# Hfx-J/SGTD

Measured on AMD Instinct MI355X. Metric: query frames/sec vs map size (descriptor build + candidate selection), higher is better.
Workload: dtype f64

## Files before the change

sgtd_amd/csrc/common.hip.h:

```cpp
#pragma once
#include <hip/hip_runtime.h>
#include <stdint.h>

#define SGTD_WAVE 64
#define SGTD_MAX_K 16
#define SGTD_NCELL 27
#define SGTD_MAX_CAND 64

typedef unsigned long long u64;
typedef unsigned int u32;

struct DevCfg {
  int K;
  int tpi;
  int cand_num;
  double min_len, max_len, scale, rough;
};

__device__ __forceinline__ int lane_id() { return threadIdx.x & (SGTD_WAVE - 1); }

__device__ __forceinline__ u64 lanemask_lt() {
  return (1ull << lane_id()) - 1ull;
}

// ... 138 lines not shown
typedef float f32x2 __attribute__((ext_vector_type(2)));

struct HashSlot {
  u64 key;
  u32 bucket;
  u32 len;
};
#define SGTD_EMPTY_KEY 0xFFFFFFFFFFFFFFFFull

__device__ __forceinline__ u32 wave_incl_scan(u32 v) {
  int x = (int)v;
  x += __builtin_amdgcn_update_dpp(0, x, 0x111, 0xf, 0xf, false);
  x += __builtin_amdgcn_update_dpp(0, x, 0x112, 0xf, 0xf, false);
  x += __builtin_amdgcn_update_dpp(0, x, 0x114, 0xf, 0xf, false);
  x += __builtin_amdgcn_update_dpp(0, x, 0x118, 0xf, 0xf, false);
  x += __builtin_amdgcn_update_dpp(0, x, 0x142, 0xa, 0xf, false);
  x += __builtin_amdgcn_update_dpp(0, x, 0x143, 0xc, 0xf, false);
  return (u32)x;
}

__device__ __forceinline__ u32 wave_sum(u32 v) {
  return (u32)__builtin_amdgcn_readlane((int)wave_incl_scan(v), SGTD_WAVE - 1);
}

__device__ __forceinline__ u32 wave_max_u32(u32 v) {
  int x = (int)v;
#define SGTD_MAX_STEP(ctrl, rows) { const u32 o = (u32)__builtin_amdgcn_update_dpp(0, x, ctrl, rows, 0xf, false); x = (int)((u32)x > o ? (u32)x : o); }
  SGTD_MAX_STEP(0x111, 0xf) SGTD_MAX_STEP(0x112, 0xf) SGTD_MAX_STEP(0x114, 0xf) SGTD_MAX_STEP(0x118, 0xf)
  SGTD_MAX_STEP(0x142, 0xa) SGTD_MAX_STEP(0x143, 0xc)
#undef SGTD_MAX_STEP
  return (u32)__builtin_amdgcn_readlane(x, SGTD_WAVE - 1);
}

template <int BITS>
__device__ __forceinline__ void wave_group_rank(u32 digit, bool valid, u32 &rank, u32 &count) {
  u64 m = __ballot(valid);
#pragma unroll
  for (int b = 0; b < BITS; b++) {
    u64 bal = __ballot((digit >> b) & 1u);
    m &= ((digit >> b) & 1u) ? bal : ~bal;
  }
  rank = __popcll(m & lanemask_lt());
  count = __popcll(m);
}
```

sgtd_amd/csrc/probe_kernels.hip.h:

```cpp
#pragma once
#include "common.hip.h"
#include <type_traits>

struct TableView {
  const HotEntry *ent;
  IdMap map;
  const double *cold_side;
  const BucketDir *dir;
  const HashSlot *hash;
  u32 hash_mask;
  u32 n_entries;
  u32 frame_lo;
  u32 frame_span;
  u32 coarse_at;
  u32 whole_at;
  u32 tail_off;
  const BucketDir *dir1;
  const HashSlot *hash1;
  u32 hash_mask1;
  u32 n_entries1;
};
__host__ __device__ __forceinline__ u32 group_row_bytes(const TableView &T) { return T.tail_off ? 2u * SGTD_GROUP_ROW_BYTES : SGTD_GROUP_ROW_BYTES; }

struct QueryView {
// ... 80 lines not shown
  for (int q0 = 0; q0 < n_queries; q0 += 256) {
    const int q = q0 + threadIdx.x;
    const u32 v = (q < n_queries) ? count[q] : 0;
    u32 tot;
    const u32 ex = block_excl_scan(v, lds, tot);
    if (q < n_queries) q_prefix[q] = carry + ex;
    carry += tot;
  }
  if (threadIdx.x == 0) *n_valid = carry;
}

__device__ __forceinline__ u64 home_coord(double s, u64 cmask) {
  return (int)(s - 1.0) < 0 ? cmask : min((u64)(u32)(int)s, cmask);
}

template <class KeyT>
__global__ void home_keys_kernel(QueryView Q, const u32 *q_prefix, KeyT *keys, u32 *vals, long long n_slots,
                                 int cbits, int sub_bits) {
  const long long d = (long long)blockIdx.x * blockDim.x + threadIdx.x;
  if (d >= n_slots) return;
  const int q = (int)(d / Q.stride);
  const u32 i = (u32)(d - (long long)q * Q.stride);
  if (i >= Q.count[q]) return;
  const u64 code = label_code(Q.label[d * 3 + 0], Q.label[d * 3 + 1], Q.label[d * 3 + 2]);
  const u64 cmask = (1ull << cbits) - 1ull;
  const u64 x = home_coord(Q.side[d * 3 + 0], cmask), y = home_coord(Q.side[d * 3 + 1], cmask),
            z = home_coord(Q.side[d * 3 + 2], cmask);
  const u32 idx = q_prefix[q] + i;
  const int ny = 1 << (sub_bits >> 1), nz = 1 << (sub_bits - (sub_bits >> 1));
  const double f1 = Q.side[d * 3 + 1] - (double)(int)Q.side[d * 3 + 1], f2 = Q.side[d * 3 + 2] - (double)(int)Q.side[d * 3 + 2];
  const u64 sub = (u64)min(max((int)(f1 * ny), 0), ny - 1) * nz + (u64)min(max((int)(f2 * nz), 0), nz - 1);
  keys[idx] = (KeyT)(((((code << cbits | x) << cbits | y) << cbits) | z) << sub_bits | sub);
  vals[idx] = (u32)d;
}

template <class KeyT>
__global__ void group_heads_kernel(const KeyT *keys, const u32 *n_valid_p, u32 *flags, long long n, int cbits, int sub_bits) {
  const long long p = (long long)blockIdx.x * blockDim.x + threadIdx.x;
  if (p >= n) return;
  u32 head = 0;
  if (p + 1 < (long long)*n_valid_p) {
    const u64 a = (u64)keys[p + 1] >> sub_bits, b = (u64)keys[p] >> sub_bits;
    const u64 cmask = (1ull << cbits) - 1ull;
    head = (a != b) || ((a & cmask) == cmask) || (((a >> cbits) & cmask) == cmask) ||
           (((a >> (2 * cbits)) & cmask) == cmask);
  }
  flags[p] = head;
}

__global__ void group_first_kernel(const u32 *gid, const u32 *n_valid_p, u32 *group_first, u32 *n_groups, long long n) {
  const long long p = (long long)blockIdx.x * blockDim.x + threadIdx.x;
  const long long nv = (long long)*n_valid_p;
  if (p >= n || p >= nv) return;
  const u32 g = gid[p];
  if (p == 0 || gid[p - 1] != g) group_first[g] = (u32)p;
  if (p == nv - 1) *n_groups = g + 1;
}

__global__ __launch_bounds__(256) void group_resolve_kernel(TableView T, QueryView Q, const u32 *order,
                                                            const u32 *group_first, const u32 *n_groups_p,
                                                            const u32 *n_valid_p, unsigned char *rows, u32 rows_cap,
                                                            int *overflow) {
  const int c = (int)(threadIdx.x & 31);
  const long long stride = ((long long)gridDim.x * blockDim.x) >> 5;
  const long long n_groups = (*n_valid_p) ? (long long)*n_groups_p : 0;
  if (n_groups > (long long)rows_cap) {
    if (blockIdx.x == 0 && threadIdx.x == 0) overflow[0] = 1;
    return;
  }
  for (long long g = ((long long)blockIdx.x * blockDim.x + threadIdx.x) >> 5; g < n_groups; g += stride) {
    if (c >= SGTD_NCELL) continue;
    const long long d = (long long)order[group_first[g]];
    const double q0 = Q.side[d * 3 + 0], q1 = Q.side[d * 3 + 1], q2 = Q.side[d * 3 + 2];
    const u32 code = label_code(Q.label[d * 3 + 0], Q.label[d * 3 + 1], Q.label[d * 3 + 2]);
    const int ix = c / 9 - 1, iy = (c / 3) % 3 - 1, iz = c % 3 - 1;
    const bool nonneg = q0 >= 0.0 && q1 >= 0.0 && q2 >= 0.0;
    const int x = nonneg ? max((int)q0 + ix, 0) : (int)(q0 + (double)ix);
    const int y = nonneg ? max((int)q1 + iy, 0) : (int)(q1 + (double)iy);
    const int z = nonneg ? max((int)q2 + iz, 0) : (int)(q2 + (double)iz);
    const bool minus_one = nonneg && ((ix < 0 && (int)(q0 + (double)ix) < 0) || (iy < 0 && (int)(q1 + (double)iy) < 0) ||
                                      (iz < 0 && (int)(q2 + (double)iz) < 0));
    const bool probe = !minus_one && x >= 0 && y >= 0 && z >= 0 && x < 65536 && y < 65536 && z < 65536;
    const u64 key = probe ? pack_key(code, (u32)x, (u32)y, (u32)z) : 0ull;
    for (int sg = 0; sg < (T.tail_off ? 2 : 1); sg++) {
      const HashSlot *hash = sg ? T.hash1 : T.hash;
      const BucketDir *dir = sg ? T.dir1 : T.dir;
      const u32 mask = sg ? T.hash_mask1 : T.hash_mask;
      uint4 lo = make_uint4(0, 0, 0, 0), hi = make_uint4(0, 0, 0, 0);
      if (probe) {
// ... 15 lines not shown
      uint4 *out = reinterpret_cast<uint4 *>(rows + (size_t)g * group_row_bytes(T) + (size_t)sg * SGTD_GROUP_ROW_BYTES);
      if (hi.w != 0u) {
        const u32 r = 1u + 2u * (u32)__builtin_popcount(exh & ((1u << c) - 1u));
        out[r] = lo;
        out[r + 1] = hi;
      }
      if (c == 0) out[0] = make_uint4(exh, (u32)(ov >> sh) & 0x7FFFFFFu, 0u, 0u);
    }
  }
}

#define SGTD_NO_PASS 0xFFFFFFFFu
#define SGTD_PASS_HDR_WORDS (SGTD_PASS_KMAX == 4 ? 32 : 16)
#define SGTD_PASS_HDR_UNITS (SGTD_PASS_HDR_WORDS / 4)
#define SGTD_META_SENTINEL (((1u << SGTD_PASS_KMAX) - 1u) << 8)
enum { PH_SLOT = 0, PH_FRAME, PH_Q0, PH_Q1, PH_Q2, PH_LO2, PH_HI2 };
__host__ __device__ constexpr int pass_hdr_word(int field, int k) { return 2 + field * SGTD_PASS_KMAX + k; }
#define SGTD_PASS_SLACK_UNITS 64

struct __attribute__((packed, aligned(4))) RangeWords { u32 offc, dlc, meta; };

struct PassPool {
  uint4 *pool;
  u32 *rec_off;
  u32 *cursor;
  u32 cap;
};

__host__ __device__ __forceinline__ u32 pass_slot_count(u32 n_valid, u32 n_groups, bool pair) {
  if (!n_valid) return 0u;
  return pair ? n_groups + (n_valid + SGTD_PAIR - 1u) / SGTD_PAIR + 1u : n_valid;
}

__global__ void pass_slots_kernel(const u32 *gid, const u32 *group_first, const u32 *n_valid_p, u32 *pos_of_slot,
                                  long long n, int pair) {
  const long long p = (long long)blockIdx.x * blockDim.x + threadIdx.x;
  if (p >= n || p >= (long long)*n_valid_p) return;
  if (!pair) { pos_of_slot[p] = (u32)p; return; }
  const u32 g = gid[p], f = group_first[g];
  if ((((u32)p - f) % SGTD_PAIR) == 0u) pos_of_slot[g + (f + SGTD_PAIR - 1u) / SGTD_PAIR + ((u32)p - f) / SGTD_PAIR] = (u32)p;
}

#define SGTD_SMALL_SLOTS 8192
#define SGTD_SMALL_THREADS 1024
struct SmallOrder {
  u32 *ctr; u32 ctr_words;
  u32 *q_M; unsigned long long *q_P;
  u32 *votes; u32 *slot_of_words; u32 span;
  int *cand_frame, *cand_votes; int cand_num;
  u32 *q_prefix, *n_valid, *order, *gid, *group_first, *n_groups, *pos_of_slot;
  u32 n_slots, max_pass_slots;
  int cbits, sub_bits, pair, key_bits;
  QueryRec *qrec; u32 n_qrec; double rough;
};
__global__ __launch_bounds__(SGTD_SMALL_THREADS) void small_order_kernel(QueryView Q, SmallOrder S) {
  extern __shared__ __attribute__((aligned(16))) unsigned char s_raw[];
  u64 *s_key = reinterpret_cast<u64 *>(s_raw);
  u32 *s_gid = reinterpret_cast<u32 *>(s_raw + SGTD_SMALL_SLOTS * 8);
  u32 *s_first = s_gid + SGTD_SMALL_SLOTS;
  __shared__ u32 s_sum[SGTD_SMALL_THREADS / SGTD_WAVE + 1];
  __shared__ u32 s_cnt[4096];
  const u32 tid = threadIdx.x;
  for (u32 i = tid; i < S.ctr_words; i += SGTD_SMALL_THREADS) S.ctr[i] = 0u;
  if (tid == 0) { S.q_M[0] = 0u; S.q_P[0] = 0ull; S.q_prefix[0] = 0u; }
  if (S.votes) for (u32 i = tid; i < S.span; i += SGTD_SMALL_THREADS) S.votes[i] = 0u;
  if (S.slot_of_words) for (u32 i = tid; i < (S.span + 3u) / 4u; i += SGTD_SMALL_THREADS) S.slot_of_words[i] = 0xFFFFFFFFu;
  if (S.cand_frame) for (u32 i = tid; i < (u32)S.cand_num; i += SGTD_SMALL_THREADS) { S.cand_frame[i] = -1; S.cand_votes[i] = 0; }
  for (u32 i = tid; i < S.max_pass_slots; i += SGTD_SMALL_THREADS) S.pos_of_slot[i] = SGTD_NO_PASS;
  if (S.qrec)
    for (u32 i = tid; i < S.n_qrec; i += SGTD_SMALL_THREADS) write_query_rec(S.qrec + i, Q.side[i * 3], Q.side[i * 3 + 1], Q.side[i * 3 + 2], S.rough, Q.frame[i]);
  const u32 nv = min(Q.count[0], S.n_slots);
  u32 P = SGTD_SMALL_THREADS;
  while (P < nv) P <<= 1;
// ... 1574 lines not shown
```

sgtd_amd/csrc/sgtd_accel.hip:

```cpp
#include "../../include/sgtd_accel.h"

#include <hip/hip_runtime.h>

#include <algorithm>
#include <atomic>
#include <chrono>
#include <cmath>
#include <cstdio>
#include <cstring>
#include <limits>
#include <memory>
#include <string>
#include <vector>

#include "build_kernel.hip.h"
#include "common.hip.h"
#include "table_kernels.hip.h"
#include "probe_kernels.hip.h"
#include "select_kernels.hip.h"
#include "verify_kernels.hip.h"
#include "verify_mfma.hip.h"
#include "exchange_kernels.hip.h"
#include "remove_kernels.hip.h"
#include "filter_kernels.hip.h"
// ... 182 lines not shown
  DevBuf v_score, v_pose, v_inlier, v_best;
  DevBuf inl_pairs, inl_off;
  bool verify_counted = false;
  DevBuf inl_counts;
  DevBuf in_block;
  size_t frame_inl_cap = 0;
  char *frame_host = nullptr;
  size_t frame_host_bytes = 0;
  DevBuf b_in, b_out;
  char *pin_build = nullptr;
  size_t pin_build_cap = 0;
  DevBuf v_hyp64, v_hyp32, v_bound;
  DevBuf v_hypB, v_tau, v_words;
  DevBuf v_okey[2], v_oval[2];
  bool verified = false;
  DevBuf r_pose, r_rmse, r_rmse_v, r_npairs, r_moments, r_flag;
  bool refined = false;
  int *export_packed = nullptr;
  size_t export_cap = 0;
  hipEvent_t ev_cand = nullptr, ev_export_free = nullptr;
  bool export_busy = false;
  u32 batch_serial = 0;
  bool defer_lists = false;
  bool lists_pending = false;
  bool lists_masked = false;
  bool fused_votes_last = false;
  const u64 *verify_keep = nullptr;
  const u64 *list_keep = nullptr;
  bool pairs_per_query = false;
  DevBuf rough_qi, rough_entry, rough_frame, rough_cell, rough_dis;
  size_t rec_cap = (size_t)1 << 25;
  bool rec_cap_fixed = false;
  size_t pair_cap = (size_t)1 << 24;
  DevBuf n_valid, cell_rows, gid, q_prefix, group_first, n_groups;
  DevBuf pos_of_slot, rec_off, pass_pool;
  size_t pool_units = 0;
  size_t group_cap = 0;
  size_t group_cap_hook = 0;
  int sorted_chunk = 0;
  bool diag = false;
  int select_mode = 0;
  PinnedVec<u32> h_count, h_pair_base, h_q_M;
  PinnedVec<unsigned long long> h_q_P;
  PinnedVec<int> h_n_cand, h_cand_frame, h_cand_votes;
  PinnedVec<long long> h_pair_off;
  sgtd_stats stats{};
  char *pin = nullptr;
  size_t pin_cap = 0, pin_used = 0;
  struct PinCopy { void *dst; size_t off, bytes; };
  std::vector<PinCopy> pin_pending;
};

#include "multi.hip.h"

namespace {

#define HIPCHK(call)                                                          \
  do {                                                                        \
    hipError_t _s = (call);                                                   \
    if (_s != hipSuccess) {                                                   \
      e->err = std::string(#call) + ": " + hipGetErrorString(_s);             \
      return SGTD_ERR_HIP;                                                    \
    }                                                                         \
  } while (0)
#define CHK(call)                 \
  do {                            \
    int _r = (call);              \
// ... 270 lines not shown
      else HIPCHK(hipMemsetAsync(dst[f], 0, bytes[f], e->stream));
    }
    CHK(ensure(e, e->in_block, bo.total));
    HIPCHK(hipMemcpyAsync(e->in_block.p, e->pin + off, bo.total, hipMemcpyHostToDevice, e->stream));
    unpack_desc_block_kernel<<<(unsigned)std::min<long long>(grid_for((long long)n * 34, 256), 512), 256, 0, e->stream>>>(e->in_block.as<unsigned char>(), (u32)n, present, s.view(),
                                                                                                                       (long long)first);
    HIPCHK(hipGetLastError());
    if (wait) CHK(xfer_sync(e));
    return SGTD_OK;
  }
#define CP(field, T, w)                                                                        \
  if (in->field)                                                                               \
    CHK(h2d(e, s.field.as<T>() + first * (w), in->field, n * (w) * sizeof(T)));               \
  else                                                                                         \
    HIPCHK(hipMemsetAsync(s.field.as<T>() + first * (w), 0, n * (w) * sizeof(T), e->stream));
  CP(side, double, 3) CP(angle, double, 3) CP(center, double, 3) CP(vertex, float, 9)
  CP(label, int, 3) CP(frame, u32, 1) CP(node_id, int, 3)
#undef CP
  if (wait) CHK(xfer_sync(e));
  return SGTD_OK;
}

void note_frames(sgtd_engine *e, u32 lo, u32 hi) {
  if (!e->have_frames) {
    e->frame_lo = lo; e->frame_hi = hi; e->have_frames = true;
  } else {
    e->frame_lo = std::min(e->frame_lo, lo);
    e->frame_hi = std::max(e->frame_hi, hi);
  }
}

template <class KeyT>
int radix_sort_pairs(sgtd_engine *e, KeyT *&kin, KeyT *&kout, u32 *&vin, u32 *&vout, long long n, int bits,
                     bool skip_const, const u32 *n_dev = nullptr) {
  const int nblocks = (int)((n + SGTD_RS_TILE - 1) / SGTD_RS_TILE);
  CHK(ensure(e, e->hist, (size_t)256 * nblocks * sizeof(u32)));
  CHK(ensure(e, e->digit_tot, 256 * sizeof(u32)));
  std::vector<u32> tot(256);
  for (int shift = 0; shift < bits; shift += 8) {
    u32 *hist = e->hist.as<u32>();
    radix_hist_kernel<KeyT><<<nblocks, SGTD_RS_THREADS, 0, e->stream>>>(kin, n, shift, hist, nblocks, n_dev);
    HIPCHK(hipGetLastError());
    if (skip_const) {
      radix_digit_totals_kernel<<<256, SGTD_SCAN_THREADS, 0, e->stream>>>(hist, nblocks, e->digit_tot.as<u32>());
      HIPCHK(hipGetLastError());
      HIPCHK(hipMemcpyAsync(tot.data(), e->digit_tot.p, 256 * sizeof(u32), hipMemcpyDeviceToHost, e->stream));
      HIPCHK(hipStreamSynchronize(e->stream));
      bool constant = false;
      for (int d = 0; d < 256; d++)
        if ((long long)tot[d] == n) constant = true;
      if (constant) continue;
    }
    CHK(device_scan(e, hist, hist, (long long)256 * nblocks));
    radix_scatter_kernel<KeyT><<<nblocks, SGTD_RS_THREADS, 0, e->stream>>>(kin, vin, kout, vout, n, shift,
                                                                       e->hist.as<u32>(), nblocks, n_dev);
    HIPCHK(hipGetLastError());
    std::swap(kin, kout);
    std::swap(vin, vout);
  }
  return SGTD_OK;
}

IdMap id_map(const sgtd_engine *e, u32 bits) {
  IdMap m;
  m.frame_first = e->frame_first.as<u32>();
  m.by_frame = e->id_by_frame ? e->by_frame.as<u32>() : nullptr;
  m.bits = bits;
  m.frame_lo = e->have_frames ? e->frame_lo : 0;
  return m;
}

int build_segment(sgtd_engine *e, sgtd_engine::Segment &S, long long g0, long long g1) {
  const long long E = g1 - g0;
  S.g0 = g0; S.g1 = g1;
  S.n_buckets = 0;
  S.hash_mask = 1023;
  S.sum_len_sq = 0.0;
  S.frame_hi = e->have_frames ? e->frame_hi : 0;
  S.built = true;
  if (E == 0) {
    CHK(ensure(e, S.hash, (size_t)1024 * sizeof(HashSlot)));
    HIPCHK(hipMemsetAsync(S.hash.p, 0xFF, (size_t)1024 * sizeof(HashSlot), e->stream));
    return SGTD_OK;
  }
  const double *side = e->tab.side.as<double>() + (size_t)g0 * 3;
  const int *label = e->tab.label.as<int>() + (size_t)g0 * 3;
  const u32 *frame = e->tab.frame.as<u32>() + (size_t)g0;
  CHK(ensure(e, e->keyA, (size_t)E * sizeof(u64)));
  CHK(ensure(e, e->keyB, (size_t)E * sizeof(u64)));
  CHK(ensure(e, e->valA, (size_t)E * sizeof(u32)));
  CHK(ensure(e, e->valB, (size_t)E * sizeof(u32)));
  CHK(ensure(e, e->bad_flag, 2 * sizeof(int)));
  HIPCHK(hipMemsetAsync(e->bad_flag.p, 0, 2 * sizeof(int), e->stream));
// ... 509 lines not shown
  CHK(ensure(e, e->cell_rows, std::max<size_t>(e->group_cap, 1) * SGTD_GROUP_ROW_BYTES * row_slots));
  const unsigned char *rows = e->cell_rows.as<unsigned char>();
  const u32 rows_cap = (u32)std::min<size_t>(e->group_cap, 0xFFFFFFFFu);
  {
    CHK(ensure(e, e->keyA, (size_t)n_slots * sizeof(u64)));
    CHK(ensure(e, e->keyB, (size_t)n_slots * sizeof(u64)));
    CHK(ensure(e, e->valA, (size_t)n_slots * sizeof(u32)));
    CHK(ensure(e, e->valB, (size_t)n_slots * sizeof(u32)));
    CHK(ensure(e, e->gid, (size_t)n_slots * sizeof(u32)));
    CHK(ensure(e, e->n_valid, sizeof(u32)));
    u64 *kin = e->keyA.as<u64>(), *kout = e->keyB.as<u64>();
    u32 *vin = e->valA.as<u32>(), *vout = e->valB.as<u32>();
    CHK(ensure(e, e->q_prefix, (size_t)nq * sizeof(u32)));
    CHK(ensure(e, e->group_first, (size_t)n_slots * sizeof(u32)));
    CHK(ensure(e, e->n_groups, sizeof(u32)));
    const bool pair = !e->diag && SGTD_PAIR >= 2;
    const size_t max_pass_slots = (size_t)pass_slot_count((u32)n_slots, (u32)n_slots, pair) + 64;
    CHK(ensure(e, e->pos_of_slot, max_pass_slots * sizeof(u32)));
    CHK(ensure(e, e->rec_off, max_pass_slots * sizeof(u32)));
    if (e->pool_units == 0) e->pool_units = std::max<size_t>(65536, (size_t)n_slots * (e->n_entries > 100000000 ? 16 : 10));
    CHK(ensure(e, e->pass_pool, (e->pool_units + SGTD_PASS_SLACK_UNITS) * sizeof(uint4)));
    const u32 *nv = e->n_valid.as<u32>();
    if (small) {
      SmallOrder SO;
      SO.ctr = e->cursors.as<u32>(); SO.ctr_words = (u32)kCtrWords;
      SO.q_M = e->q_M.as<u32>(); SO.q_P = e->q_P.as<unsigned long long>();
      SO.votes = votes_per_query ? nullptr : e->votes.as<u32>(); SO.slot_of_words = e->slot_of.as<u32>(); SO.span = span;
      SO.cand_frame = e->cand_frame.as<int>(); SO.cand_votes = e->cand_votes.as<int>(); SO.cand_num = cn;
      SO.q_prefix = e->q_prefix.as<u32>(); SO.n_valid = e->n_valid.as<u32>(); SO.order = vin; SO.gid = e->gid.as<u32>();
      SO.group_first = e->group_first.as<u32>(); SO.n_groups = e->n_groups.as<u32>(); SO.pos_of_slot = e->pos_of_slot.as<u32>();
      SO.n_slots = (u32)n_slots; SO.max_pass_slots = (u32)max_pass_slots; SO.cbits = cbits; SO.sub_bits = sub_bits; SO.pair = pair ? 1 : 0; SO.key_bits = key_bits;
      SO.qrec = nullptr; SO.n_qrec = 0; SO.rough = e->dc.rough;
      const size_t lds = (size_t)SGTD_SMALL_SLOTS * 16;
      static const bool lds_set = [&] { return hipFuncSetAttribute(reinterpret_cast<const void *>(&small_order_kernel), hipFuncAttributeMaxDynamicSharedMemorySize, (int)lds) == hipSuccess; }();
      if (!lds_set) return SGTD_ERR_HIP;
      small_order_kernel<<<1, SGTD_SMALL_THREADS, lds, e->stream>>>(v.Q, SO);
      HIPCHK(hipGetLastError());
    } else {
    query_prefix_kernel<<<1, 256, 0, e->stream>>>(e->q_count.as<u32>(), e->q_prefix.as<u32>(), nq, e->n_valid.as<u32>());
    HIPCHK(hipGetLastError());
    if (key_bits <= 32) {
      u32 *k32 = reinterpret_cast<u32 *>(kin), *k32o = reinterpret_cast<u32 *>(kout);
      home_keys_kernel<u32><<<grid_for(n_slots, 256), 256, 0, e->stream>>>(v.Q, e->q_prefix.as<u32>(), k32, vin, n_slots, cbits, sub_bits);
      HIPCHK(hipGetLastError());
      CHK(radix_sort_pairs(e, k32, k32o, vin, vout, n_slots, key_bits, false, nv));
      group_heads_kernel<u32><<<grid_for(n_slots, 256), 256, 0, e->stream>>>(k32, nv, e->gid.as<u32>(), n_slots, cbits, sub_bits);
    } else {
      home_keys_kernel<u64><<<grid_for(n_slots, 256), 256, 0, e->stream>>>(v.Q, e->q_prefix.as<u32>(), kin, vin, n_slots, cbits, sub_bits);
      HIPCHK(hipGetLastError());
      CHK(radix_sort_pairs(e, kin, kout, vin, vout, n_slots, key_bits, false, nv));
      group_heads_kernel<u64><<<grid_for(n_slots, 256), 256, 0, e->stream>>>(kin, nv, e->gid.as<u32>(), n_slots, cbits, sub_bits);
    }
    HIPCHK(hipGetLastError());
    CHK(device_scan(e, e->gid.as<u32>(), e->gid.as<u32>(), n_slots));
    group_first_kernel<<<grid_for(n_slots, 256), 256, 0, e->stream>>>(e->gid.as<u32>(), nv, e->group_first.as<u32>(),
                                                                        e->n_groups.as<u32>(), n_slots);
    HIPCHK(hipGetLastError());
    HIPCHK(hipMemsetAsync(e->pos_of_slot.p, 0xFF, max_pass_slots * sizeof(u32), e->stream));
    pass_slots_kernel<<<grid_for(n_slots, 256), 256, 0, e->stream>>>(e->gid.as<u32>(), e->group_first.as<u32>(), nv,
                                                                       e->pos_of_slot.as<u32>(), n_slots, pair ? 1 : 0);
    HIPCHK(hipGetLastError());
    }
    e->thr2_pending = 0;
    u32 chunk = 2;
    if (e->stats.last_D > 0 && e->stats.last_P_swept > 0) {
      const double per_pass = (double)e->stats.last_P_swept / ((double)e->stats.last_D / (pair ? (SGTD_PAIR >= 4 ? 3.2 : 1.9) : 1.0));
      chunk = (u32)std::min(8.0, std::max(1.0, std::floor(1536.0 / per_pass + 0.5)));
    }
    if (e->sorted_chunk > 0) chunk = (u32)std::min(SGTD_TICKET_MAX, e->sorted_chunk);
    int sgrid = e->n_cus * 8;
    if (const char *o = getenv("SGTD_SWEEP_BLOCKS_PER_CU")) sgrid = e->n_cus * std::max(1, atoi(o));
    PassPool PP;
    PP.pool = e->pass_pool.as<uint4>(); PP.rec_off = e->rec_off.as<u32>();
    PP.cursor = v.B.pool_cursor(); PP.cap = (u32)std::min<size_t>(e->pool_units, 0xFFFFFF00u);
    {
      Views &vs = v;
      group_resolve_kernel<<<e->n_cus * 16, 256, 0, e->stream>>>(vs.T, vs.Q, vin, e->group_first.as<u32>(),
                                                                  e->n_groups.as<u32>(), nv, e->cell_rows.as<unsigned char>(), rows_cap, vs.B.overflow());
      HIPCHK(hipGetLastError());
      int plan_per_cu = 20;
      if (const char *o = getenv("SGTD_PLAN_BLOCKS_PER_CU")) plan_per_cu = std::max(1, atoi(o));
      const int pgrid = (int)std::min<long long>(grid_for((long long)max_pass_slots, SGTD_PLAN_THREADS), (long long)e->n_cus * plan_per_cu);
#define SGTD_LAUNCH_PLAN(PR, TL)                                                                               \
  plan_passes_kernel<PR, TL><<<pgrid, SGTD_PLAN_THREADS, 0, e->stream>>>(vs.T, vs.Q, vin, e->gid.as<u32>(), e->pos_of_slot.as<u32>(), nv, \
                                                       e->n_groups.as<u32>(), rows, rows_cap, PP, vs.B.n_visit, vs.B.list,          \
                                                       vs.B.overflow())
      if (vs.T.tail_off) { if (pair) SGTD_LAUNCH_PLAN(true, true); else SGTD_LAUNCH_PLAN(false, true); }
      else { if (pair) SGTD_LAUNCH_PLAN(true, false); else SGTD_LAUNCH_PLAN(false, false); }
#undef SGTD_LAUNCH_PLAN
      HIPCHK(hipGetLastError());
      if (e->timing) HIPCHK(hipEventRecord(e->ev[EV_SORT], e->stream));
      const bool narrow = ((unsigned long long)vs.T.n_entries + SGTD_SENTINELS + (vs.T.tail_off ? vs.T.n_entries1 + SGTD_SENTINELS : 0u)) * sizeof(HotEntry) < (1ull << 32);
      const bool frames = e->last_kind != 1 || (e->have_frames && e->last_qframe >= e->frame_lo && e->last_qframe <= e->frame_hi);
// ... 2035 lines not shown
```

sgtd_amd/csrc/table_kernels.hip.h:

```cpp
#pragma once
#include "common.hip.h"

#define SGTD_SCAN_THREADS 256
#define SGTD_SCAN_ITEMS 8

__device__ __forceinline__ u32 block_excl_scan(u32 v, u32 *lds_wave , u32 &block_total) {
  const int lane = lane_id(), wid = threadIdx.x >> 6, nw = blockDim.x >> 6;
  u32 inc = wave_incl_scan(v);
  if (lane == SGTD_WAVE - 1) lds_wave[wid] = inc;
  __syncthreads();
  if (wid == 0) {
    u32 w = (lane < nw) ? lds_wave[lane] : 0;
    u32 wi = wave_incl_scan(w);
    if (lane < nw) lds_wave[lane] = wi - w;
    if (lane == nw - 1) lds_wave[nw] = wi;
  }
  __syncthreads();
  u32 r = lds_wave[wid] + inc - v;
  block_total = lds_wave[nw];
  __syncthreads();
  return r;
}

__global__ __launch_bounds__(SGTD_SCAN_THREADS) void scan_reduce_kernel(const u32 *in, u32 *block_sums, long long n) {
// ... 40 lines not shown
  if ((unsigned)x > 65535u || (unsigned)y > 65535u || (unsigned)z > 65535u) {
    *bad_flag = 1;
    x &= 65535; y &= 65535; z &= 65535;
  }
  keys[g] = pack_key(label_code(label[g * 3], label[g * 3 + 1], label[g * 3 + 2]), (u32)x, (u32)y, (u32)z);
  vals[g] = (u32)g;
}

__global__ void frame_keys_kernel(const u32 *frame, u64 *keys, u32 *vals, long long n) {
  long long g = (long long)blockIdx.x * blockDim.x + threadIdx.x;
  if (g >= n) return;
  keys[g] = frame[g];
  vals[g] = (u32)g;
}
__global__ void keys_of_order_kernel(const double *side, const int *label, const u32 *order, u64 *keys, long long n) {
  long long p = (long long)blockIdx.x * blockDim.x + threadIdx.x;
  if (p >= n) return;
  const size_t g = order[p];
  const int x = (int)(side[g * 3 + 0] + 0.5), y = (int)(side[g * 3 + 1] + 0.5), z = (int)(side[g * 3 + 2] + 0.5);
  keys[p] = pack_key(label_code(label[g * 3], label[g * 3 + 1], label[g * 3 + 2]), (u32)x & 65535u, (u32)y & 65535u, (u32)z & 65535u);
}

__global__ void frame_range_check_kernel(const u32 *frame, long long n, u32 lo, u32 hi, int *bad_flag) {
  long long g = (long long)blockIdx.x * blockDim.x + threadIdx.x;
  if (g < n && (frame[g] < lo || frame[g] > hi)) *bad_flag = 1;
}

#define SGTD_RS_THREADS 256
#define SGTD_RS_ROUNDS 16
#define SGTD_RS_TILE (SGTD_RS_THREADS * SGTD_RS_ROUNDS)

template <class KeyT>
__global__ __launch_bounds__(SGTD_RS_THREADS) void radix_hist_kernel(const KeyT *keys, long long n, int shift,
                                                                      u32 *hist, int nblocks,
                                                                      const u32 *n_dev = nullptr) {
  __shared__ u32 h[256];
  if (n_dev) n = min(n, (long long)*n_dev);
  h[threadIdx.x] = 0;
  __syncthreads();
  long long base = (long long)blockIdx.x * SGTD_RS_TILE;
#pragma unroll 4
  for (int r = 0; r < SGTD_RS_ROUNDS; r++) {
    long long i = base + (long long)r * SGTD_RS_THREADS + threadIdx.x;
    if (i < n) atomicAdd(&h[(u32)(keys[i] >> shift) & 255u], 1u);
  }
  __syncthreads();
  hist[(size_t)threadIdx.x * nblocks + blockIdx.x] = h[threadIdx.x];
}

__global__ void radix_digit_totals_kernel(const u32 *hist, int nblocks, u32 *tot) {
  __shared__ u32 lds[SGTD_SCAN_THREADS / SGTD_WAVE + 1];
  const int d = blockIdx.x;
  u32 s = 0;
  for (int b = threadIdx.x; b < nblocks; b += blockDim.x) s += hist[(size_t)d * nblocks + b];
  u32 t;
  block_excl_scan(s, lds, t);
  if (threadIdx.x == 0) tot[d] = t;
}

template <class KeyT>
__global__ __launch_bounds__(SGTD_RS_THREADS) void radix_scatter_kernel(
    const KeyT *keys_in, const u32 *vals_in, KeyT *keys_out, u32 *vals_out, long long n,
    int shift, const u32 *hist_scanned, int nblocks, const u32 *n_dev = nullptr) {
  constexpr int NW = SGTD_RS_THREADS / SGTD_WAVE;
  __shared__ u32 run[256];
  __shared__ u32 wcount[NW][256];
  const int tid = threadIdx.x, wid = tid >> 6;
  if (n_dev) n = min(n, (long long)*n_dev);
  if ((long long)blockIdx.x * SGTD_RS_TILE >= n) return;
  run[tid] = hist_scanned[(size_t)tid * nblocks + blockIdx.x];
  long long base = (long long)blockIdx.x * SGTD_RS_TILE;
  for (int r = 0; r < SGTD_RS_ROUNDS; r++) {
#pragma unroll
    for (int w = 0; w < NW; w++) wcount[w][tid] = 0;
    __syncthreads();
    long long i = base + (long long)r * SGTD_RS_THREADS + tid;
    const bool valid = i < n;
    KeyT k = valid ? keys_in[i] : 0;
    u32 v = valid ? vals_in[i] : 0;
    u32 digit = (u32)(k >> shift) & 255u;
    u32 rank, count;
    wave_group_rank<8>(digit, valid, rank, count);
    if (valid && rank == 0) wcount[wid][digit] = count;
    __syncthreads();
    if (valid) {
      u32 pos = run[digit] + rank;
#pragma unroll
      for (int w = 0; w < NW; w++)
        if (w < wid) pos += wcount[w][digit];
      keys_out[pos] = k;
      vals_out[pos] = v;
    }
    __syncthreads();
    u32 add = 0;
#pragma unroll
    for (int w = 0; w < NW; w++) add += wcount[w][tid];
    run[tid] += add;
  }
}

__global__ void gather_hot_kernel(u32 *perm, const double *side, const u32 *frame, const u32 *id_of_g, IdMap map,
                                  HotEntry *ent, long long n, u32 g0) {
  long long p = (long long)blockIdx.x * blockDim.x + threadIdx.x;
  if (p >= n) {
    if (p < n + SGTD_SENTINELS) {
      HotEntry h;
      h.s0 = h.s1 = h.s2 = __builtin_inff();
      h.id = SGTD_DEAD_ID;
      ent[p] = h;
      perm[p] = 0;
    }
    return;
  }
  const u32 g = perm[p];
  perm[p] = g + g0;
  HotEntry h;
  h.s0 = (float)side[(size_t)g * 3 + 0];
  h.s1 = (float)side[(size_t)g * 3 + 1];
  h.s2 = (float)side[(size_t)g * 3 + 2];
  if (id_of_g) h.id = id_of_g[g + g0];
  else {
    const u32 f = frame[g] - map.frame_lo;
    h.id = (f << map.bits) | ((g + g0) - map.frame_first[f]);
  }
  ent[p] = h;
}

__global__ void frame_first_kernel(const u32 *key, long long n, u32 lo, u32 *first) {
  long long p = (long long)blockIdx.x * blockDim.x + threadIdx.x;
  if (p >= n) return;
// ... 284 lines not shown
```

Measured before the change: 184,600.

## Size radix sort and grouping grids to live count with fused group pass

Replaces the candidate-sort path with live-count-aware radix kernels. Each pass uses a persistent grid sized from last frame's observed slot count and loops only over live tiles, with a per-digit row scan in place of the full device scan. The grouping stage (heads, scan, first, memset, pass slots) becomes two kernels, per-block parts and apply, which compute gid, group_first, n_groups and pos_of_slot in one sweep. This cuts launches and the work spent on the padded n_slots capacity, in exchange for more complex kernels and a grid-size heuristic based on earlier statistics.

```diff
diff --git a/sgtd_amd/csrc/common.hip.h b/sgtd_amd/csrc/common.hip.h
--- a/sgtd_amd/csrc/common.hip.h
+++ b/sgtd_amd/csrc/common.hip.h
@@ -194,6 +194,15 @@
   return (u32)__builtin_amdgcn_readlane(x, SGTD_WAVE - 1);
 }
 
+__device__ __forceinline__ u32 wave_incl_max_scan(u32 v) {
+  int x = (int)v;
+#define SGTD_MAX_STEP(ctrl, rows) { const u32 o = (u32)__builtin_amdgcn_update_dpp(0, x, ctrl, rows, 0xf, false); x = (int)((u32)x > o ? (u32)x : o); }
+  SGTD_MAX_STEP(0x111, 0xf) SGTD_MAX_STEP(0x112, 0xf) SGTD_MAX_STEP(0x114, 0xf) SGTD_MAX_STEP(0x118, 0xf)
+  SGTD_MAX_STEP(0x142, 0xa) SGTD_MAX_STEP(0x143, 0xc)
+#undef SGTD_MAX_STEP
+  return (u32)x;
+}
+
 template <int BITS>
 __device__ __forceinline__ void wave_group_rank(u32 digit, bool valid, u32 &rank, u32 &count) {
   u64 m = __ballot(valid);
diff --git a/sgtd_amd/csrc/probe_kernels.hip.h b/sgtd_amd/csrc/probe_kernels.hip.h
--- a/sgtd_amd/csrc/probe_kernels.hip.h
+++ b/sgtd_amd/csrc/probe_kernels.hip.h
@@ -136,29 +136,6 @@
   const u64 sub = (u64)min(max((int)(f1 * ny), 0), ny - 1) * nz + (u64)min(max((int)(f2 * nz), 0), nz - 1);
   keys[idx] = (KeyT)(((((code << cbits | x) << cbits | y) << cbits) | z) << sub_bits | sub);
   vals[idx] = (u32)d;
-}
-
-template <class KeyT>
-__global__ void group_heads_kernel(const KeyT *keys, const u32 *n_valid_p, u32 *flags, long long n, int cbits, int sub_bits) {
-  const long long p = (long long)blockIdx.x * blockDim.x + threadIdx.x;
-  if (p >= n) return;
-  u32 head = 0;
-  if (p + 1 < (long long)*n_valid_p) {
-    const u64 a = (u64)keys[p + 1] >> sub_bits, b = (u64)keys[p] >> sub_bits;
-    const u64 cmask = (1ull << cbits) - 1ull;
-    head = (a != b) || ((a & cmask) == cmask) || (((a >> cbits) & cmask) == cmask) ||
-           (((a >> (2 * cbits)) & cmask) == cmask);
-  }
-  flags[p] = head;
-}
-
-__global__ void group_first_kernel(const u32 *gid, const u32 *n_valid_p, u32 *group_first, u32 *n_groups, long long n) {
-  const long long p = (long long)blockIdx.x * blockDim.x + threadIdx.x;
-  const long long nv = (long long)*n_valid_p;
-  if (p >= n || p >= nv) return;
-  const u32 g = gid[p];
-  if (p == 0 || gid[p - 1] != g) group_first[g] = (u32)p;
-  if (p == nv - 1) *n_groups = g + 1;
 }
 
 __global__ __launch_bounds__(256) void group_resolve_kernel(TableView T, QueryView Q, const u32 *order,
@@ -240,13 +217,113 @@
   return pair ? n_groups + (n_valid + SGTD_PAIR - 1u) / SGTD_PAIR + 1u : n_valid;
 }
 
-__global__ void pass_slots_kernel(const u32 *gid, const u32 *group_first, const u32 *n_valid_p, u32 *pos_of_slot,
-                                  long long n, int pair) {
-  const long long p = (long long)blockIdx.x * blockDim.x + threadIdx.x;
-  if (p >= n || p >= (long long)*n_valid_p) return;
-  if (!pair) { pos_of_slot[p] = (u32)p; return; }
-  const u32 g = gid[p], f = group_first[g];
-  if ((((u32)p - f) % SGTD_PAIR) == 0u) pos_of_slot[g + (f + SGTD_PAIR - 1u) / SGTD_PAIR + ((u32)p - f) / SGTD_PAIR] = (u32)p;
+#define SGTD_GROUP_THREADS 256
+#define SGTD_GROUP_ITEMS 16
+#define SGTD_GROUP_BLOCK (SGTD_GROUP_THREADS * SGTD_GROUP_ITEMS)
+template <class KeyT>
+__device__ __forceinline__ bool group_starts(KeyT prev, KeyT cur, int cbits, int sub_bits) {
+  const u64 a = (u64)cur >> sub_bits, b = (u64)prev >> sub_bits;
+  const u64 cmask = (1ull << cbits) - 1ull;
+  return (a != b) || ((a & cmask) == cmask) || (((a >> cbits) & cmask) == cmask) || (((a >> (2 * cbits)) & cmask) == cmask);
+}
+__device__ __forceinline__ u32 block_max_u32(u32 m, u32 *lds_wave) {
+  const int wid = threadIdx.x >> 6, nw = blockDim.x >> 6;
+  const u32 wm = wave_max_u32(m);
+  if (lane_id() == 0) lds_wave[wid] = wm;
+  __syncthreads();
+  u32 r = 0;
+  for (int w = 0; w < nw; w++) r = max(r, lds_wave[w]);
+  __syncthreads();
+  return r;
+}
+
+template <class KeyT>
+__global__ __launch_bounds__(SGTD_GROUP_THREADS) void group_parts_kernel(const KeyT *keys, const u32 *n_valid_p, long long n_cap,
+                                                                          uint2 *parts, int cbits, int sub_bits) {
+  __shared__ u32 lds[SGTD_GROUP_THREADS / SGTD_WAVE + 1];
+  const long long nv = min(n_cap, (long long)*n_valid_p);
+  const int live = (int)((nv + SGTD_GROUP_BLOCK - 1) / SGTD_GROUP_BLOCK);
+  for (int blk = blockIdx.x; blk < live; blk += gridDim.x) {
+    const long long p0 = (long long)blk * SGTD_GROUP_BLOCK + (long long)threadIdx.x * SGTD_GROUP_ITEMS;
+    u32 cnt = 0, last = 0;
+    KeyT prev = (p0 > 0 && p0 - 1 < nv) ? keys[p0 - 1] : (KeyT)0;
+#pragma unroll
+    for (int k = 0; k < SGTD_GROUP_ITEMS; k++) {
+      const long long p = p0 + k;
+      const KeyT cur = p < nv ? keys[p] : (KeyT)0;
+      if (p < nv && (p == 0 || group_starts(prev, cur, cbits, sub_bits))) { cnt++; last = (u32)p + 1u; }
+      prev = cur;
+    }
+    u32 tot;
+    block_excl_scan(cnt, lds, tot);
+    const u32 mx = block_max_u32(last, lds);
+    if (threadIdx.x == 0) parts[blk] = make_uint2(tot, mx);
+  }
+}
+
+template <class KeyT>
+__global__ __launch_bounds__(SGTD_GROUP_THREADS) void group_apply_kernel(const KeyT *keys, const u32 *n_valid_p, long long n_cap,
+                                                                          const uint2 *parts, int cbits, int sub_bits, int pair,
+                                                                          u32 *gid, u32 *group_first, u32 *n_groups, u32 *pos_of_slot) {
+  __shared__ u32 lds[SGTD_GROUP_THREADS / SGTD_WAVE + 1];
+  const long long nv = min(n_cap, (long long)*n_valid_p);
+  const int live = (int)((nv + SGTD_GROUP_BLOCK - 1) / SGTD_GROUP_BLOCK);
+  const int lane = lane_id(), wid = threadIdx.x >> 6;
+  for (int blk = blockIdx.x; blk < live; blk += gridDim.x) {
+    u32 c_before = 0, f_before = 0;
+    for (int j = threadIdx.x; j < blk; j += SGTD_GROUP_THREADS) {
+      const uint2 t = parts[j];
+      c_before += t.x; f_before = max(f_before, t.y);
+    }
+    u32 tot;
+    block_excl_scan(c_before, lds, tot);
+    c_before = tot;
+    f_before = block_max_u32(f_before, lds);
+    const long long p0 = (long long)blk * SGTD_GROUP_BLOCK + (long long)threadIdx.x * SGTD_GROUP_ITEMS;
+    u32 st = 0;
+    KeyT prev = (p0 > 0 && p0 - 1 < nv) ? keys[p0 - 1] : (KeyT)0;
+#pragma unroll
+    for (int k = 0; k <= SGTD_GROUP_ITEMS; k++) {
+      const long long p = p0 + k;
+      const KeyT cur = p < nv ? keys[p] : (KeyT)0;
+      if (p < nv && (p == 0 || group_starts(prev, cur, cbits, sub_bits))) st |= 1u << k;
+      prev = cur;
+    }
+    const u32 mine = st & ((1u << SGTD_GROUP_ITEMS) - 1u);
+    const u32 cnt = (u32)__builtin_popcount(mine);
+    const u32 last = mine ? (u32)p0 + (31u - (u32)__builtin_clz(mine)) + 1u : 0u;
+    u32 g = c_before + block_excl_scan(cnt, lds, tot);
+    const u32 inc = wave_incl_max_scan(last);
+    if (lane == SGTD_WAVE - 1) lds[wid] = inc;
+    __syncthreads();
+    u32 f = f_before;
+    for (int w = 0; w < wid; w++) f = max(f, lds[w]);
+    const u32 up = (u32)__builtin_amdgcn_update_dpp(0, (int)inc, 0x138, 0xf, 0xf, false);
+    f = max(f, lane ? up : 0u);
+    __syncthreads();
+#pragma unroll
+    for (int k = 0; k < SGTD_GROUP_ITEMS; k++) {
+      const long long pl = p0 + k;
+      if (pl >= nv) continue;
+      const u32 p = (u32)pl;
+      if ((st >> k) & 1u) { g++; f = p + 1u; group_first[g - 1u] = p; }
+      const u32 gi = g - 1u, fp = f - 1u;
+      gid[p] = gi;
+      const bool ends = pl + 1 >= nv || ((st >> (k + 1)) & 1u);
+      if (!pair) pos_of_slot[p] = p;
+      else {
+        const u32 s0 = gi + (fp + SGTD_PAIR - 1u) / SGTD_PAIR;
+        if (((p - fp) % SGTD_PAIR) == 0u) pos_of_slot[s0 + (p - fp) / SGTD_PAIR] = p;
+        if (ends) {
+          const u32 next = pl + 1 >= nv ? pass_slot_count((u32)nv, gi + 1u, true) : gi + 1u + (p + 1u + SGTD_PAIR - 1u) / SGTD_PAIR;
+          const u32 s1 = s0 + (p - fp) / SGTD_PAIR + 1u;
+          if (s1 < next) pos_of_slot[s1] = SGTD_NO_PASS;
+          if (s1 + 1u < next) pos_of_slot[s1 + 1u] = SGTD_NO_PASS;
+        }
+      }
+      if (pl + 1 >= nv) *n_groups = gi + 1u;
+    }
+  }
 }
 
 #define SGTD_SMALL_SLOTS 8192
diff --git a/sgtd_amd/csrc/sgtd_accel.hip b/sgtd_amd/csrc/sgtd_accel.hip
--- a/sgtd_amd/csrc/sgtd_accel.hip
+++ b/sgtd_amd/csrc/sgtd_accel.hip
@@ -238,7 +238,7 @@
   size_t rec_cap = (size_t)1 << 25;
   bool rec_cap_fixed = false;
   size_t pair_cap = (size_t)1 << 24;
-  DevBuf n_valid, cell_rows, gid, q_prefix, group_first, n_groups;
+  DevBuf n_valid, cell_rows, gid, q_prefix, group_first, n_groups, group_parts;
   DevBuf pos_of_slot, rec_off, pass_pool;
   size_t pool_units = 0;
   size_t group_cap = 0;
@@ -575,14 +575,14 @@
 
 template <class KeyT>
 int radix_sort_pairs(sgtd_engine *e, KeyT *&kin, KeyT *&kout, u32 *&vin, u32 *&vout, long long n, int bits,
-                     bool skip_const, const u32 *n_dev = nullptr) {
+                     bool skip_const) {
   const int nblocks = (int)((n + SGTD_RS_TILE - 1) / SGTD_RS_TILE);
   CHK(ensure(e, e->hist, (size_t)256 * nblocks * sizeof(u32)));
   CHK(ensure(e, e->digit_tot, 256 * sizeof(u32)));
   std::vector<u32> tot(256);
   for (int shift = 0; shift < bits; shift += 8) {
     u32 *hist = e->hist.as<u32>();
-    radix_hist_kernel<KeyT><<<nblocks, SGTD_RS_THREADS, 0, e->stream>>>(kin, n, shift, hist, nblocks, n_dev);
+    radix_hist_kernel<KeyT><<<nblocks, SGTD_RS_THREADS, 0, e->stream>>>(kin, n, shift, hist, nblocks);
     HIPCHK(hipGetLastError());
     if (skip_const) {
       radix_digit_totals_kernel<<<256, SGTD_SCAN_THREADS, 0, e->stream>>>(hist, nblocks, e->digit_tot.as<u32>());
@@ -596,12 +596,40 @@
     }
     CHK(device_scan(e, hist, hist, (long long)256 * nblocks));
     radix_scatter_kernel<KeyT><<<nblocks, SGTD_RS_THREADS, 0, e->stream>>>(kin, vin, kout, vout, n, shift,
-                                                                       e->hist.as<u32>(), nblocks, n_dev);
+                                                                       e->hist.as<u32>(), nblocks);
     HIPCHK(hipGetLastError());
     std::swap(kin, kout);
     std::swap(vin, vout);
   }
   return SGTD_OK;
+}
+
+template <class KeyT>
+int radix_sort_pairs_live(sgtd_engine *e, KeyT *&kin, KeyT *&kout, u32 *&vin, u32 *&vout, long long n_cap, int bits,
+                          const u32 *n_dev, int grid_tiles) {
+  const int nblocks = (int)((n_cap + SGTD_RS_TILE - 1) / SGTD_RS_TILE);
+  CHK(ensure(e, e->hist, (size_t)256 * nblocks * sizeof(u32)));
+  CHK(ensure(e, e->digit_tot, 256 * sizeof(u32)));
+  const int grid = std::max(1, std::min(nblocks, grid_tiles));
+  u32 *hist = e->hist.as<u32>(), *tot = e->digit_tot.as<u32>();
+  for (int shift = 0; shift < bits; shift += 8) {
+    radix_hist_live_kernel<KeyT><<<grid, SGTD_RS_THREADS, 0, e->stream>>>(kin, n_cap, shift, hist, nblocks, n_dev);
+    radix_digit_scan_kernel<<<256, SGTD_SCAN_THREADS, 0, e->stream>>>(hist, nblocks, n_cap, n_dev, tot);
+    radix_scatter_live_kernel<KeyT><<<grid, SGTD_RS_THREADS, 0, e->stream>>>(kin, vin, kout, vout, n_cap, shift, hist, nblocks, tot, n_dev);
+    HIPCHK(hipGetLastError());
+    std::swap(kin, kout);
+    std::swap(vin, vout);
+  }
+  return SGTD_OK;
+}
+
+int live_grid(const sgtd_engine *e, long long n_slots, long long per) {
+  long long n = n_slots;
+  if (e->stats.last_queries > 0 && e->stats.last_D > 0) {
+    const double guess = (double)e->stats.last_D / (double)e->stats.last_queries * (double)e->nq;
+    n = std::min<long long>(n_slots, (long long)(guess * 1.0625) + per);
+  }
+  return (int)std::max<long long>(1, (n + per - 1) / per);
 }
 
 IdMap id_map(const sgtd_engine *e, u32 bits) {
@@ -1177,33 +1205,35 @@
       SO.n_slots = (u32)n_slots; SO.max_pass_slots = (u32)max_pass_slots; SO.cbits = cbits; SO.sub_bits = sub_bits; SO.pair = pair ? 1 : 0; SO.key_bits = key_bits;
       SO.qrec = nullptr; SO.n_qrec = 0; SO.rough = e->dc.rough;
       const size_t lds = (size_t)SGTD_SMALL_SLOTS * 16;
-      static const bool lds_set = [&] { return hipFuncSetAttribute(reinterpret_cast<const void *>(&small_order_kernel), hipFuncAttributeMaxDynamicSharedMemorySize, (int)lds) == hipSuccess; }();
-      if (!lds_set) return SGTD_ERR_HIP;
+      HIPCHK(hipFuncSetAttribute(reinterpret_cast<const void *>(&small_order_kernel), hipFuncAttributeMaxDynamicSharedMemorySize, (int)lds));
       small_order_kernel<<<1, SGTD_SMALL_THREADS, lds, e->stream>>>(v.Q, SO);
       HIPCHK(hipGetLastError());
     } else {
     query_prefix_kernel<<<1, 256, 0, e->stream>>>(e->q_count.as<u32>(), e->q_prefix.as<u32>(), nq, e->n_valid.as<u32>());
     HIPCHK(hipGetLastError());
+    const int sort_grid = live_grid(e, n_slots, SGTD_RS_TILE), group_grid = live_grid(e, n_slots, SGTD_GROUP_BLOCK);
+    CHK(ensure(e, e->group_parts, (size_t)((n_slots + SGTD_GROUP_BLOCK - 1) / SGTD_GROUP_BLOCK) * sizeof(uint2)));
+    uint2 *parts = e->group_parts.as<uint2>();
+#define SGTD_LAUNCH_GROUPS(KEYS)                                                                                              \
+  do {                                                                                                                        \
+    group_parts_kernel<<<group_grid, SGTD_GROUP_THREADS, 0, e->stream>>>(KEYS, nv, n_slots, parts, cbits, sub_bits);          \
+    group_apply_kernel<<<group_grid, SGTD_GROUP_THREADS, 0, e->stream>>>(KEYS, nv, n_slots, parts, cbits, sub_bits, pair ? 1 : 0, \
+                                                                         e->gid.as<u32>(), e->group_first.as<u32>(),          \
+                                                                         e->n_groups.as<u32>(), e->pos_of_slot.as<u32>());    \
+  } while (0)
     if (key_bits <= 32) {
       u32 *k32 = reinterpret_cast<u32 *>(kin), *k32o = reinterpret_cast<u32 *>(kout);
       home_keys_kernel<u32><<<grid_for(n_slots, 256), 256, 0, e->stream>>>(v.Q, e->q_prefix.as<u32>(), k32, vin, n_slots, cbits, sub_bits);
       HIPCHK(hipGetLastError());
-      CHK(radix_sort_pairs(e, k32, k32o, vin, vout, n_slots, key_bits, false, nv));
-      group_heads_kernel<u32><<<grid_for(n_slots, 256), 256, 0, e->stream>>>(k32, nv, e->gid.as<u32>(), n_slots, cbits, sub_bits);
+      CHK(radix_sort_pairs_live(e, k32, k32o, vin, vout, n_slots, key_bits, nv, sort_grid));
+      SGTD_LAUNCH_GROUPS(k32);
     } else {
       home_keys_kernel<u64><<<grid_for(n_slots, 256), 256, 0, e->stream>>>(v.Q, e->q_prefix.as<u32>(), kin, vin, n_slots, cbits, sub_bits);
       HIPCHK(hipGetLastError());
-      CHK(radix_sort_pairs(e, kin, kout, vin, vout, n_slots, key_bits, false, nv));
-      group_heads_kernel<u64><<<grid_for(n_slots, 256), 256, 0, e->stream>>>(kin, nv, e->gid.as<u32>(), n_slots, cbits, sub_bits);
-    }
-    HIPCHK(hipGetLastError());
-    CHK(device_scan(e, e->gid.as<u32>(), e->gid.as<u32>(), n_slots));
-    group_first_kernel<<<grid_for(n_slots, 256), 256, 0, e->stream>>>(e->gid.as<u32>(), nv, e->group_first.as<u32>(),
-                                                                        e->n_groups.as<u32>(), n_slots);
-    HIPCHK(hipGetLastError());
-    HIPCHK(hipMemsetAsync(e->pos_of_slot.p, 0xFF, max_pass_slots * sizeof(u32), e->stream));
-    pass_slots_kernel<<<grid_for(n_slots, 256), 256, 0, e->stream>>>(e->gid.as<u32>(), e->group_first.as<u32>(), nv,
-                                                                       e->pos_of_slot.as<u32>(), n_slots, pair ? 1 : 0);
+      CHK(radix_sort_pairs_live(e, kin, kout, vin, vout, n_slots, key_bits, nv, sort_grid));
+      SGTD_LAUNCH_GROUPS(kin);
+    }
+#undef SGTD_LAUNCH_GROUPS
     HIPCHK(hipGetLastError());
     }
     e->thr2_pending = 0;
diff --git a/sgtd_amd/csrc/table_kernels.hip.h b/sgtd_amd/csrc/table_kernels.hip.h
--- a/sgtd_amd/csrc/table_kernels.hip.h
+++ b/sgtd_amd/csrc/table_kernels.hip.h
@@ -96,10 +96,8 @@
 
 template <class KeyT>
 __global__ __launch_bounds__(SGTD_RS_THREADS) void radix_hist_kernel(const KeyT *keys, long long n, int shift,
-                                                                      u32 *hist, int nblocks,
-                                                                      const u32 *n_dev = nullptr) {
+                                                                      u32 *hist, int nblocks) {
   __shared__ u32 h[256];
-  if (n_dev) n = min(n, (long long)*n_dev);
   h[threadIdx.x] = 0;
   __syncthreads();
   long long base = (long long)blockIdx.x * SGTD_RS_TILE;
@@ -125,13 +123,11 @@
 template <class KeyT>
 __global__ __launch_bounds__(SGTD_RS_THREADS) void radix_scatter_kernel(
     const KeyT *keys_in, const u32 *vals_in, KeyT *keys_out, u32 *vals_out, long long n,
-    int shift, const u32 *hist_scanned, int nblocks, const u32 *n_dev = nullptr) {
+    int shift, const u32 *hist_scanned, int nblocks) {
   constexpr int NW = SGTD_RS_THREADS / SGTD_WAVE;
   __shared__ u32 run[256];
   __shared__ u32 wcount[NW][256];
   const int tid = threadIdx.x, wid = tid >> 6;
-  if (n_dev) n = min(n, (long long)*n_dev);
-  if ((long long)blockIdx.x * SGTD_RS_TILE >= n) return;
   run[tid] = hist_scanned[(size_t)tid * nblocks + blockIdx.x];
   long long base = (long long)blockIdx.x * SGTD_RS_TILE;
   for (int r = 0; r < SGTD_RS_ROUNDS; r++) {
@@ -160,6 +156,107 @@
 #pragma unroll
     for (int w = 0; w < NW; w++) add += wcount[w][tid];
     run[tid] += add;
+  }
+}
+
+__device__ __forceinline__ int radix_live_tiles(long long n_cap, const u32 *n_dev) {
+  const long long n = min(n_cap, (long long)*n_dev);
+  return (int)((n + SGTD_RS_TILE - 1) / SGTD_RS_TILE);
+}
+
+template <class KeyT>
+__global__ __launch_bounds__(SGTD_RS_THREADS) void radix_hist_live_kernel(const KeyT *keys, long long n_cap, int shift,
+                                                                           u32 *hist, int nblocks, const u32 *n_dev) {
+  __shared__ u32 h[256];
+  const long long n = min(n_cap, (long long)*n_dev);
+  const int live = radix_live_tiles(n_cap, n_dev);
+  for (int tile = blockIdx.x; tile < live; tile += gridDim.x) {
+    h[threadIdx.x] = 0;
+    __syncthreads();
+    const long long base = (long long)tile * SGTD_RS_TILE;
+#pragma unroll 4
+    for (int r = 0; r < SGTD_RS_ROUNDS; r++) {
+      const long long i = base + (long long)r * SGTD_RS_THREADS + threadIdx.x;
+      if (i < n) atomicAdd(&h[(u32)(keys[i] >> shift) & 255u], 1u);
+    }
+    __syncthreads();
+    hist[(size_t)threadIdx.x * nblocks + tile] = h[threadIdx.x];
+  }
+}
+
+__global__ __launch_bounds__(SGTD_SCAN_THREADS) void radix_digit_scan_kernel(u32 *hist, int nblocks, long long n_cap,
+                                                                              const u32 *n_dev, u32 *tot) {
+  __shared__ u32 lds[SGTD_SCAN_THREADS / SGTD_WAVE + 1];
+  const int live = radix_live_tiles(n_cap, n_dev);
+  u32 *row = hist + (size_t)blockIdx.x * nblocks;
+  u32 carry = 0;
+  for (int b0 = 0; b0 < live; b0 += SGTD_SCAN_THREADS * SGTD_SCAN_ITEMS) {
+    u32 v[SGTD_SCAN_ITEMS];
+    u32 s = 0;
+#pragma unroll
+    for (int k = 0; k < SGTD_SCAN_ITEMS; k++) {
+      const int i = b0 + (int)threadIdx.x * SGTD_SCAN_ITEMS + k;
+      v[k] = (i < live) ? row[i] : 0;
+      s += v[k];
+    }
+    u32 t;
+    u32 ex = block_excl_scan(s, lds, t) + carry;
+#pragma unroll
+    for (int k = 0; k < SGTD_SCAN_ITEMS; k++) {
+      const int i = b0 + (int)threadIdx.x * SGTD_SCAN_ITEMS + k;
+      if (i < live) row[i] = ex;
+      ex += v[k];
+    }
+    carry += t;
+  }
+  if (threadIdx.x == 0) tot[blockIdx.x] = carry;
+}
+
+template <class KeyT>
+__global__ __launch_bounds__(SGTD_RS_THREADS) void radix_scatter_live_kernel(
+    const KeyT *keys_in, const u32 *vals_in, KeyT *keys_out, u32 *vals_out, long long n_cap,
+    int shift, const u32 *hist_scanned, int nblocks, const u32 *digit_tot, const u32 *n_dev) {
+  constexpr int NW = SGTD_RS_THREADS / SGTD_WAVE;
+  __shared__ u32 run[256];
+  __shared__ u32 wcount[NW][256];
+  __shared__ u32 lds[NW + 1];
+  const int tid = threadIdx.x, wid = tid >> 6;
+  const long long n = min(n_cap, (long long)*n_dev);
+  const int live = radix_live_tiles(n_cap, n_dev);
+  u32 all;
+  const u32 digit_base = block_excl_scan(digit_tot[tid], lds, all);
+  for (int tile = blockIdx.x; tile < live; tile += gridDim.x) {
+    run[tid] = digit_base + hist_scanned[(size_t)tid * nblocks + tile];
+    const long long base = (long long)tile * SGTD_RS_TILE;
+    for (int r = 0; r < SGTD_RS_ROUNDS; r++) {
+      if (base + (long long)r * SGTD_RS_THREADS >= n) break;
+#pragma unroll
+      for (int w = 0; w < NW; w++) wcount[w][tid] = 0;
+      __syncthreads();
+      const long long i = base + (long long)r * SGTD_RS_THREADS + tid;
+      const bool valid = i < n;
+      const KeyT k = valid ? keys_in[i] : 0;
+      const u32 v = valid ? vals_in[i] : 0;
+      const u32 digit = (u32)(k >> shift) & 255u;
+      u32 rank, count;
+      wave_group_rank<8>(digit, valid, rank, count);
+      if (valid && rank == 0) wcount[wid][digit] = count;
+      __syncthreads();
+      if (valid) {
+        u32 pos = run[digit] + rank;
+#pragma unroll
+        for (int w = 0; w < NW; w++)
+          if (w < wid) pos += wcount[w][digit];
+        keys_out[pos] = k;
+        vals_out[pos] = v;
+      }
+      __syncthreads();
+      u32 add = 0;
+#pragma unroll
+      for (int w = 0; w < NW; w++) add += wcount[w][tid];
+      run[tid] += add;
+    }
+    __syncthreads();
   }
 }
 
```

Result: no change. 186,000 (median of 6 runs) (+0.7%).
